# kennychenfs/KataCoffee

Measured on AMD Instinct MI355X. Metric: self-play training rows/sec + MCTS playouts/sec, 5x5 Coffee b6c96 @600 visits, higher is better.
Workload: dtype fp16

## Files before the change

### katacoffee_amd/csrc/search.hip

```cpp
#include <hip/hip_runtime.h>
#include <hip/hip_ext.h>

#include <type_traits>

#include "detmath.h"
#include "engine.h"
#include "kc_board.h"
#include "search.h"

namespace kc {

static constexpr int SVB_IDX_MOVE1 = MAX_P + 1;
static constexpr int SVB_IDX_PLA = 2 * (MAX_P + 1);
static constexpr int SVB_IDX_PAT = 2 * (MAX_P + 1) + 3;
static constexpr int BIG = 0x7fffffff;

KC_D int64_t svbQ(float x) { return llrintf(x * 4294967296.0f); }
KC_D float svbF(int64_t v) { return (float)v * (1.0f / 4294967296.0f); }

KC_D void waveSync() {
  __builtin_amdgcn_wave_barrier();
  asm volatile("" ::: "memory");
}

#ifdef KC_SEARCH_PROFILE
constexpr int SPROF_N = 48;
constexpr int SPROF_MAXG = 16384;
__device__ unsigned long long g_searchProf[SPROF_MAXG * SPROF_N];
__device__ unsigned long long* g_probeKeys = nullptr;
__device__ unsigned long long g_probeMask = 0;
KC_D void probeLeafKey(uint64_t k0, uint64_t k1) {
  if(!g_probeKeys)
    return;
  uint64_t key = (k0 ^ (k1 * 0x9e3779b97f4a7c15ULL)) | 1ull;
  uint64_t i = (key >> 7) & g_probeMask;
  for(int probe = 0; probe < 64; probe++, i = (i + 1) & g_probeMask) {
    const unsigned long long prev = atomicCAS(&g_probeKeys[i], 0ull, (unsigned long long)key);
    if(prev == 0ull)
      return;
    if(prev == key) {
      atomicAdd(&g_searchProf[9], 1ull);
      return;
    }
  }
}
KC_D unsigned long long* sprofLds() {
  __shared__ unsigned long long c[SPROF_N];
  return c;
}
#define SPROF_NOW() clock64()
#define SPROF_WAIT() __builtin_amdgcn_s_waitcnt(0)
#define SPROF_INIT()                   \
  do {                                 \
    if(laneId() < SPROF_N)             \
      sprofLds()[laneId()] = 0;        \
    __syncthreads();                   \
  } while(0)
#define SPROF_ADD(i, v)                                 \
  do {                                                  \
    if(laneId() == 0)                                   \
      sprofLds()[(i)] += (unsigned long long)(v);       \
  } while(0)
#define SPROF_FLUSH()                                                           \
  do {                                                                          \
    __syncthreads();                                                            \
    if(blockIdx.x < SPROF_MAXG && (laneId() < 24 || (laneId() >= 32 && laneId() < 40))) \
      g_searchProf[blockIdx.x * SPROF_N + laneId()] += sprofLds()[laneId()];    \
  } while(0)
#define SPROF_MAX(i, v)                                                                   \
  do {                                                                                    \
    if(laneId() == 0 && blockIdx.x < SPROF_MAXG) {                                        \
      unsigned long long* q_ = &g_searchProf[blockIdx.x * SPROF_N + (i)];                 \
      const unsigned long long v_ = (unsigned long long)(v);                              \
      if(v_ > *q_)                                                                        \
        *q_ = v_;                                                                         \
    }                                                                                     \
  } while(0)
#else
#define SPROF_NOW() 0ull
#define SPROF_WAIT() \
  do {               \
  } while(0)
#define SPROF_INIT() \
  do {               \
  } while(0)
#define SPROF_ADD(i, v) \
  do {                  \
  } while(0)
#define SPROF_MAX(i, v) \
  do {                  \
  } while(0)
#define SPROF_FLUSH() \
  do {                \
  } while(0)
#endif

struct NodeEdges {
  Edge* inl;
  Edge* pool;
  KC_D Edge& operator[](int i) const { return i < INLINE_EDGES ? inl[i] : pool[i - INLINE_EDGES]; }
};

struct GV {
  const SearchDev& d;
  const DTables& T;
  int g, lane;
  const SP* sp;
  const Unc* unc;
  mutable int esel = 0;
  int row;
  int32_t* wpn = nullptr;
  int32_t* wps = nullptr;
  KC_D GV(const SearchDev& d_, int g_) : d(d_), T(*d_.T), g(g_), lane(laneId()), sp(&d_.sp), unc(&d_.unc), row(g_) {}
  KC_D GV(const SearchDev& d_, const DTables& t_, int g_)
      : d(d_), T(t_), g(g_), lane(laneId()), sp(&d_.sp), unc(&d_.unc), row(g_) {}
  KC_D void setDescent(int j) {
    row = g * d.wideK + j;
    wpn = d.widePathNode + (size_t)row * MAX_DEPTH;
    wps = d.widePathSlot + (size_t)row * MAX_DEPTH;
  }
  KC_D Node* nodes() const { return d.nodes + (size_t)g * d.cap; }
  KC_D Edge* inlineEdges(int n) const { return d.edges + ((size_t)g * d.cap + n) * INLINE_EDGES; }
  KC_D Edge* edgePool() const { return d.edgePool + ((size_t)g * 2 + esel) * d.edgePoolCap; }
  KC_D void setEdgeSel(int sel) const { esel = __builtin_amdgcn_readfirstlane(sel); }
  KC_D NodeEdges edges(int n, uint32_t ebase) const { return NodeEdges{inlineEdges(n), edgePool() + ebase}; }
  KC_D NodeEdges edges(int n) const { return edges(n, nodes()[n].edgeBase); }
  KC_D uint64_t* nodeKey(int n) const { return d.nodeKey + ((size_t)g * d.cap + n) * 2; }
  KC_D float* pol(int n) const { return d.policy + ((size_t)g * d.cap + n) * d.P; }
  KC_D uint32_t* freeList() const { return d.freeList + (size_t)g * d.cap; }
  KC_D uint32_t* allocBits() const { return d.allocBits + (size_t)g * (d.cap / 32); }
  KC_D uint64_t* ttKey() const { return d.ttKey + (size_t)g * d.ttCap * 2; }
  KC_D int32_t* ttNode() const { return d.ttNode + (size_t)g * d.ttCap; }
  KC_D size_t svbBase(int sel) const { return ((size_t)g * 2 + sel) * d.svbCap; }
  KC_D float* accPolicy() const { return d.accPolicy + (size_t)g * d.P; }
  KC_D float* rawPolicy() const { return d.rawPolicy + (size_t)g * d.P; }
  KC_D float* rootNoised() const { return d.rootNoised + (size_t)g * d.P; }
  KC_D int32_t* pathNode() const { return wpn ? wpn : d.pathNode + (size_t)g * MAX_DEPTH; }
  KC_D int32_t* pathSlot() const { return wps ? wps : d.pathSlot + (size_t)g * MAX_DEPTH; }
  KC_D TurnRec* turns() const { return d.turns + (size_t)g * d.maxTurns; }
  KC_D int16_t* turnPol(int t) const { return d.turnPol + ((size_t)g * d.maxTurns + t) * d.P; }
};

static_assert(sizeof(GameDev) % 4 == 0, "GameDev copy granularity");
KC_D void storeGame(const GV& v, const GameDev& s) {
  waveSync();
  const uint32_t* src = reinterpret_cast<const uint32_t*>(&s);
  uint32_t* dst = reinterpret_cast<uint32_t*>(&v.d.games[v.g]);
  for(int i = v.lane; i < (int)(sizeof(GameDev) / 4); i += 64)
    dst[i] = src[i];
}

KC_D int sideOf(const SearchDev& d, int g, const GameDev& s) {
  return matchNet(d.slotBase + g, s.gameNum, s.root.pla);
}

template <bool MATCH = false>
KC_D void bindGame(GV& v, const GameDev& s) {
  v.sp = __builtin_amdgcn_readfirstlane(s.noNoise) ? &v.d.spCheap : &v.d.sp;
  if constexpr(MATCH) {
    if(v.d.matchPerSide && __builtin_amdgcn_readfirstlane(sideOf(v.d, v.g, s))) {
      v.sp = &v.d.sp1;
      v.unc = &v.d.unc1;
    }
  }
  v.setEdgeSel(s.edgeSel);
}

KC_D const Expl& explOf(const GV& v) { return v.unc == &v.d.unc1 ? v.d.ex1 : v.d.ex; }
KC_D const RootSearch& rootSearchOf(const GV& v) { return v.unc == &v.d.unc1 ? v.d.rs1 : v.d.rs; }

template <bool MATCH>
KC_D void matchMoveLimits(const GV& v, GameDev& s) {
  if constexpr(MATCH) {
    if(v.d.matchPerSide && __builtin_amdgcn_readfirstlane(sideOf(v.d, v.g, s)))
      s.visitLimit = v.d.sp1.maxVisits;
  }
}

template <bool MATCH = false>
KC_D void loadGame(GV& v, GameDev& s) {
  const uint32_t* src = reinterpret_cast<const uint32_t*>(&v.d.games[v.g]);
  uint32_t* dst = reinterpret_cast<uint32_t*>(&s);
  for(int i = v.lane; i < (int)(sizeof(GameDev) / 4); i += 64)
    dst[i] = src[i];
  waveSync();
  bindGame<MATCH>(v, s);
}

template <int NI>
KC_D float tsum(const float (&x)[NI], int n, int lane) {
  float a = 0.0f;
#pragma unroll
  for(int j = 0; j < NI; j++) {
    int i = lane + 64 * j;
    if(i < n)
      a = j == 0 ? x[j] : a + x[j];
  }
  return waveSum(a);
}

KC_D int bcastI(int v, int srcLane) { return bcastLane(v, srcLane); }

constexpr int SPEC_EDGES = INLINE_EDGES;
template <int NI>
constexpr bool W1_OF = NI <= 4;
KC_D int firstLane(uint64_t m) { return __builtin_ctzll(m); }

KC_D float childWeight(uint32_t edgeVisits, uint32_t childVisits, float rawWeight) {
  return rawWeight * ((float)edgeVisits / (float)(childVisits > 1u ? childVisits : 1u));
}

constexpr int PROBE_W = 16;
KC_D int ttFind(const GV& v, uint64_t k0, uint64_t k1, int& emptySlot) {
  const int mask = v.d.ttCap - 1;
  const int start = (int)(k0 & (uint64_t)mask);
  const uint64_t* key = v.ttKey();
  const int32_t* node = v.ttNode();
  emptySlot = -1;
  const bool act = v.lane < PROBE_W;
  for(int base = 0; base < v.d.ttCap; base += PROBE_W) {
    int s = (start + base + v.lane) & mask;
    const int nd = act ? node[s] : 0;
    const uint64_t ka = act ? key[2 * s] : 0ull, kb = act ? key[2 * s + 1] : 0ull;
    bool match = act && nd >= 0 && ka == k0 && kb == k1;
    uint64_t m = ballot(act && (nd < 0 || match));
    if(m) {
      int f = firstLane(m);
      emptySlot = bcastI(s, f);
      return bcastI(match ? nd : -1, f);
    }
  }
  return -1;
}

KC_D void ttInsertAt(const GV& v, int slot, uint64_t k0, uint64_t k1, int nodeIdx) {
  if(slot >= 0 && v.lane == 0) {
    v.ttKey()[2 * slot] = k0;
    v.ttKey()[2 * slot + 1] = k1;
    v.ttNode()[slot] = nodeIdx;
  }
}

KC_D uint64_t svbProbe(const GV& v, int sel, uint64_t k) {
  const int mask = v.d.svbCap - 1;
  return v.lane < PROBE_W ? v.d.svbKey[v.svbBase(sel) + (((int)(k & (uint64_t)mask) + v.lane) & mask)] : 0ull;
}
KC_D int svbFindOrInsert(const GV& v, int sel, uint64_t k, uint64_t first) {
  const int mask = v.d.svbCap - 1;
  const size_t b = v.svbBase(sel);
  const int start = (int)(k & (uint64_t)mask);
  const bool act = v.lane < PROBE_W;
  for(int base = 0; base < v.d.svbCap; base += PROBE_W) {
    int s = (start + base + v.lane) & mask;
    uint64_t kk = base == 0 ? first : (act ? v.d.svbKey[b + s] : 0ull);
    uint64_t m = ballot(act && (kk == 0 || kk == k));
    if(m) {
      int f = firstLane(m);
      int slot = bcastI(s, f);
      bool empty = bcastLane((int)(kk == 0), f) != 0;
      if(empty && v.lane == f) {
        v.d.svbKey[b + slot] = k;
        v.d.svbD[b + slot] = 0;
        v.d.svbW[b + slot] = 0;
      }
      return slot;
    }
  }
  return -1;
}

template <bool W1 = false>
KC_D uint64_t svbKeyOf(const GV& v, const DBoard& before, int parentPrevPos, int movePos, int mover) {
  const DTables& T = v.T;
  uint64_t h = 0;
  if(v.lane < 25) {
    int wy = v.lane / 5, wx = v.lane % 5;
    int cell = movePos % T.A;
    int xx = cell % T.X + wx - 2, yy = cell / T.X + wy - 2;
    int col = (xx >= 0 && xx < T.X && yy >= 0 && yy < T.Y) ? colorAt<W1>(before, yy * T.X + xx) : 3;
    h = T.svbZ[SVB_IDX_PAT + col * 25 + wy * 5 + wx];
  }
  h = waveXor64(h);
  h ^= T.svbZ[parentPrevPos] ^ T.svbZ[SVB_IDX_MOVE1 + movePos] ^ T.svbZ[SVB_IDX_PLA + mover];
  return h != 0 ? h : 1;
}

KC_D int allocNode(const GV& v, GameDev& s, int nextPla, uint64_t k0, uint64_t k1, bool terminal, int freeIdx = -1) {
  if(s.freeTop <= 0) {
    s.err = ERR_NODE_POOL;
    return -1;
  }
  s.freeTop--;
  int idx = freeIdx >= 0 ? freeIdx : (int)v.freeList()[s.freeTop];
  if(v.lane == 0) {
    Node n;
    n.visits = 0;
    n.weightSum = n.weightSqSum = n.utilityAvg = n.utilitySqAvg = n.winLossAvg = 0.0f;
    n.nnWin = n.nnLoss = n.lastSvbDelta = n.lastSvbWeight = 0.0f;
    n.svbEntry = -1;
    n.numChildren = 0;
    n.nextPla = (uint8_t)nextPla;
    n.flags = terminal ? 2 : 0;
    n.nextPrior = -1.0f;
    n.nextPos = 0xFFFF;
    n.virtualLosses = 0;
    n.edgeBase = 0;
    n.nnWeight = 1.0f;
    v.nodes()[idx] = n;
    v.nodeKey(idx)[0] = k0;
    v.nodeKey(idx)[1] = k1;
    atomicOr(&v.allocBits()[idx >> 5], 1u << (idx & 31));
  }
  s.liveCount++;
  return idx;
}

struct NStats {
  uint32_t visits;
  float weightSum, weightSqSum, utilityAvg, utilitySqAvg, winLossAvg;
};

KC_D NStats addLeafValue(const GV& v, const GameDev& s, int ni, float wl, float weight, bool isTerminal,
                         bool assumeNoExisting) {
  const SP& sp = *v.sp;
  Node* np = &v.nodes()[ni];
  const int svbEntry = np->svbEntry;
  uint32_t visits = np->visits;
  float weightSum = np->weightSum, weightSqSum = np->weightSqSum;
  float utilityAvg = np->utilityAvg, utilitySqAvg = np->utilitySqAvg, winLossAvg = np->winLossAvg;
  float utility = wl;
  if(sp.svbFactor != 0.0f && !isTerminal && svbEntry >= 0) {
    size_t e = v.svbBase(s.svbSel) + svbEntry;
    float dd = svbF(v.d.svbD[e]), ww = svbF(v.d.svbW[e]);
    if(ww > 0.001f)
      utility = utility + (sp.svbFactor * dd) / ww;
  }
  float usq = utility * utility;
  if(assumeNoExisting) {
    winLossAvg = wl;
    utilityAvg = utility;
    utilitySqAvg = usq;
    weightSqSum = weight * weight;
    weightSum = weight;
    visits += 1;
  } else {
    float oldW = weightSum, newW = oldW + weight;
    winLossAvg = (winLossAvg * oldW + wl * weight) / newW;
    utilityAvg = (utilityAvg * oldW + utility * weight) / newW;
    utilitySqAvg = (utilitySqAvg * oldW + usq * weight) / newW;
    weightSqSum = weightSqSum + weight * weight;
    weightSum = newW;
    visits += 1;
  }
  waveSync();
  if(v.lane == 0) {
    np->visits = visits;
    np->weightSum = weightSum;
    np->weightSqSum = weightSqSum;
    np->utilityAvg = utilityAvg;
    np->utilitySqAvg = utilitySqAvg;
    np->winLossAvg = winLossAvg;
  }
  waveSync();
  return NStats{visits, weightSum, weightSqSum, utilityAvg, utilitySqAvg, winLossAvg};
}

KC_D float cdfT(const DTables& T, float z) {
  float dd = (1999.0f * (z - (-50.0f))) / 100.0f;
  if(dd <= 0.0f)
    return 0.0f;
  int idx = (int)dd;
  if(idx >= 1999)
    return 1.0f;
  float lambda = dd - (float)idx;
  float y0 = T.cdf[idx], y1 = T.cdf[idx + 1];
  return y0 + lambda * (y1 - y0);
}

template <int NI, bool EXPL>
struct PathPriors {};
template <int NI>
struct PathPriors<NI, true> {
  float epr[NI];
};
template <int NI, bool EXPL = false>
struct PathLevel : PathPriors<NI, EXPL> {
  int ni, slot, k, nextPla, svbEntry;
  uint32_t ebase;
  float nnWin, nnLoss, nnWeight, lastSvbDelta, lastSvbWeight;
  uint32_t visits0;
  uint32_t ech[NI], evis[NI];
  uint32_t cv[NI];
  float cws[NI], cwsq[NI], cu[NI], cusq[NI], cwl[NI];
  int64_t svbD0, svbW0;
};
struct LevelOut {
  NStats st;
  int svbEntry;
  int64_t svbD, svbW;
};

template <int NI, bool EXPL>
KC_D void loadLevel(const GV& v, int ni, int slot, PathLevel<NI, EXPL>& L) {
  const Node nd = v.nodes()[ni];
  const Edge* E = v.inlineEdges(ni);
  const Edge e0 = v.lane < SPEC_EDGES && v.lane < v.d.P ? E[v.lane] : Edge{0u, 0u, 0.0f, 0u};
  L.ebase = nd.edgeBase;
  L.ech[0] = e0.child;
  L.evis[0] = e0.visits;
  L.ni = ni;
  L.slot = slot;
  L.k = nd.numChildren;
  L.nextPla = nd.nextPla;
  L.svbEntry = nd.svbEntry;
  L.nnWin = nd.nnWin;
  L.nnLoss = nd.nnLoss;
  L.nnWeight = nd.nnWeight;
  L.lastSvbDelta = nd.lastSvbDelta;
  L.lastSvbWeight = nd.lastSvbWeight;
  L.visits0 = nd.visits;
}

template <int NI, bool EXPL>
KC_D void loadKids(const GV& v, const GameDev& s, PathLevel<NI, EXPL>& L) {
  const SP& sp = *v.sp;
  const NodeEdges E = v.edges(L.ni, L.ebase);
  const Node* NS = v.nodes();
#pragma unroll
  for(int j = 0; j < NI; j++) {
    const int i = v.lane + 64 * j;
    L.cv[j] = 0;
    L.cws[j] = L.cwsq[j] = L.cu[j] = L.cusq[j] = L.cwl[j] = 0.0f;
    if constexpr(EXPL)
      L.epr[j] = 0.0f;
    if(j > 0 || i >= SPEC_EDGES)
      L.ech[j] = L.evis[j] = 0u;
    if(i < L.k) {
      if(j > 0 || i >= SPEC_EDGES) {
        const Edge e = E[i];
        L.ech[j] = e.child;
        L.evis[j] = e.visits;
      }
      if constexpr(EXPL) {
        const Edge e = E[i];
        L.epr[j] = L.ni == s.rootIdx ? v.rootNoised()[e.move] : e.prior;
      }
      const Node& c = NS[L.ech[j]];
      L.cv[j] = c.visits;
      L.cws[j] = c.weightSum;
      L.cwsq[j] = c.weightSqSum;
      L.cu[j] = c.utilityAvg;
      L.cusq[j] = c.utilitySqAvg;
      L.cwl[j] = c.winLossAvg;
    }
  }
  const size_t e = v.svbBase(s.svbSel) + (L.svbEntry >= 0 ? L.svbEntry : 0);
  L.svbD0 = v.d.svbD[e];
  L.svbW0 = v.d.svbW[e];
  (void)sp;
}

template <int NI, bool EXPL, class F>
KC_D LevelOut computeLevel(const GV& v, const GameDev& s, PathLevel<NI, EXPL>& L, const LevelOut& below, bool haveBelow,
                           int numVisitsToAdd, bool isRoot, F&& issueNext) {
  const SP& sp = *v.sp;
  const unsigned long long tLoads = SPROF_NOW();
  (void)tLoads;
  SPROF_WAIT();
  const unsigned long long tCalc = SPROF_NOW();
  (void)tCalc;
  SPROF_ADD(36, tCalc - tLoads);
  SPROF_ADD(39, 1);
  const int k = L.k, slot = L.slot;
  const int nextPla = L.nextPla;
  const int svbEntry = L.svbEntry;
  const NodeEdges E = v.edges(L.ni, L.ebase);
  const bool svbOn = sp.svbFactor != 0.0f && svbEntry >= 0;
  int64_t svbD0 = L.svbD0, svbW0 = L.svbW0;
  if(svbOn && haveBelow && below.svbEntry == svbEntry) {
    svbD0 = below.svbD;
    svbW0 = below.svbW;
  }
  bool good[NI];
  float wAdj[NI], selfU[NI], cU[NI], cUsq[NI], cWl[NI], cWs[NI], cWsq[NI], tmp[NI];
  int numGood = 0;
  float maxW = 0.0f;
#pragma unroll
  for(int j = 0; j < NI; j++) {
    int i = v.lane + 64 * j;
    good[j] = false;
    wAdj[j] = selfU[j] = cU[j] = cUsq[j] = cWl[j] = cWs[j] = cWsq[j] = 0.0f;
    if(i < k) {
      uint32_t evis = L.evis[j];
      uint32_t cv = L.cv[j];
      float ws = L.cws[j], wsq = L.cwsq[j], u = L.cu[j], usq = L.cusq[j], wl = L.cwl[j];
      if(i == slot) {
        evis += 1;
        E[i].visits = evis;
        if(haveBelow) {
          cv = below.st.visits;
          ws = below.st.weightSum;
          wsq = below.st.weightSqSum;
          u = below.st.utilityAvg;
          usq = below.st.utilitySqAvg;
          wl = below.st.winLossAvg;
        }
      }
      good[j] = cv > 0 && ws > 0.0f && evis > 0;
      if(good[j]) {
        cU[j] = u;
        cUsq[j] = usq;
        cWl[j] = wl;
        cWs[j] = ws;
        cWsq[j] = wsq;
        selfU[j] = nextPla == 2 ? cU[j] : -cU[j];
        wAdj[j] = childWeight(evis, cv, ws);
        maxW = wAdj[j] > maxW ? wAdj[j] : maxW;
      }
    }
    numGood += __popcll(ballot(good[j]));
  }
  maxW = waveMax(maxW);
  const float origTotal = tsum<NI>(wAdj, k, v.lane);
  float currentTotal = origTotal;
  bool pruning = false;
  if constexpr(EXPL) {
    const Expl& ex = explOf(v);
    pruning = ex.noisePruning != 0;
    if(pruning && pruneNoiseApplies(numGood, origTotal)) {
      PruneScan sc{0.0f, 0.0f, 0.0f};
#pragma unroll
      for(int j = 0; j < NI; j++) {
        const int cnt = k - 64 * j < 64 ? k - 64 * j : 64;
        const uint64_t gm = ballot(good[j]);
        for(int l = 0; l < cnt; l++) {
          if(!((gm >> l) & 1ull))
            continue;
          const float old = bcastLaneF(wAdj[j], l), u = bcastLaneF(selfU[j], l), pr = bcastLaneF(L.epr[j], l);
          const float nw = pruneNoiseStep(ex, sc, old, u, pr);
          if(v.lane == l)
            wAdj[j] = nw;
        }
      }
      currentTotal = sc.wSum;
    }
  }
  float amountToSubtract = 0.0f, amountToPrune = 0.0f;
  if(isRoot && sp.rootNoise && !pruning) {
    amountToSubtract = fminf(sp.moveSubtract, maxW / 64.0f);
    amountToPrune = fminf(sp.movePrune, maxW / 64.0f);
  }
  if(numGood > 0 && currentTotal > 0.0f) {
    float stdev[NI];
#pragma unroll
    for(int j = 0; j < NI; j++) {
      if(j > 0 && 64 * j >= k) {
        stdev[j] = tmp[j] = 0.0f;
        continue;
      }
      stdev[j] = good[j] ? sqrtf(1e-8f + 1.0f / (1.5f * sqrtf(wAdj[j]))) : 0.0f;
      tmp[j] = good[j] ? selfU[j] * wAdj[j] : 0.0f;
    }
    const float simpleValue = tsum<NI>(tmp, k, v.lane) / currentTotal;
    float y0[NI], y1[NI], lam[NI], pc[NI];
    int mode[NI];
#pragma unroll
    for(int j = 0; j < NI; j++) {
      mode[j] = 0;
      y0[j] = y1[j] = lam[j] = pc[j] = 0.0f;
      if(j > 0 && 64 * j >= k)
        continue;
      if(!good[j] || wAdj[j] < amountToPrune)
        continue;
      float z = (selfU[j] - simpleValue) / stdev[j];
      float dd = (1999.0f * (z - (-50.0f))) / 100.0f;
      if(dd <= 0.0f) {
        mode[j] = 2;
        pc[j] = 0.0f;
        continue;
      }
      int idx = (int)dd;
      if(idx >= 1999) {
        mode[j] = 2;
        pc[j] = 1.0f;
        continue;
      }
      mode[j] = 1;
      lam[j] = dd - (float)idx;
      y0[j] = v.T.cdf[idx];
      y1[j] = v.T.cdf[idx + 1];
    }
    issueNext();
#pragma unroll
    for(int j = 0; j < NI; j++) {
      if((j > 0 && 64 * j >= k) || mode[j] == 0) {
        tmp[j] = 0.0f;
        continue;
      }
      float nw = wAdj[j] - amountToSubtract;
      if(nw <= 0.0f)
        nw = 0.0f;
      const float c = mode[j] == 1 ? y0[j] + lam[j] * (y1[j] - y0[j]) : pc[j];
      float p = c + 0.0001f;
      float f = sp.valueWeightExp == 0.5f ? sqrtf(p) : dpow(p, sp.valueWeightExp);
      tmp[j] = nw * f;
    }
    const float totalNew = tsum<NI>(tmp, k, v.lane);
    const float factor = currentTotal / totalNew;
#pragma unroll
    for(int j = 0; j < NI; j++)
      wAdj[j] = tmp[j] * factor;
  } else {
    issueNext();
  }
  float wlv[NI], uv[NI], usqv[NI], wsqv[NI];
#pragma unroll
  for(int j = 0; j < NI; j++) {
    if((j > 0 && 64 * j >= k) || !good[j]) {
      wlv[j] = uv[j] = usqv[j] = wsqv[j] = 0.0f;
      continue;
    }
    float ws = wAdj[j] / cWs[j];
    wlv[j] = wAdj[j] * cWl[j];
    uv[j] = wAdj[j] * cU[j];
    usqv[j] = wAdj[j] * cUsq[j];
    wsqv[j] = (ws * ws) * cWsq[j];
  }
  float winLossSum = tsum<NI>(wlv, k, v.lane);
  float utilitySum = tsum<NI>(uv, k, v.lane);
  float utilitySqSum = tsum<NI>(usqv, k, v.lane);
  float weightSqSum = tsum<NI>(wsqv, k, v.lane);
  float weightSum = currentTotal;
  float wl = L.nnWin - L.nnLoss;
  float utility = wl;
  float newLastD = L.lastSvbDelta, newLastW = L.lastSvbWeight;
  LevelOut out;
  out.svbEntry = -1;
  out.svbD = out.svbW = 0;
  if(svbOn) {
    int64_t D = svbD0, Wt = svbW0;
    if(currentTotal > 1e-10f) {
      float utilityChildren = utilitySum / currentTotal;
      float svbWv = dpow(origTotal, sp.svbExp);
      float svbDv = (utilityChildren - utility) * svbWv;
      D += svbQ(svbDv) - svbQ(L.lastSvbDelta);
      Wt += svbQ(svbWv) - svbQ(L.lastSvbWeight);
      waveSync();
      if(v.lane == 0) {
        const size_t e = v.svbBase(s.svbSel) + svbEntry;
        v.d.svbD[e] = D;
        v.d.svbW[e] = Wt;
      }
      newLastD = svbDv;
      newLastW = svbWv;
      out.svbEntry = svbEntry;
      out.svbD = D;
      out.svbW = Wt;
    }
    float dd = svbF(D), ww = svbF(Wt);
    if(ww > 0.001f)
      utility = utility + (sp.svbFactor * dd) / ww;
  }
  const float selfW = L.nnWeight;
  winLossSum = winLossSum + wl * selfW;
  utilitySum = utilitySum + utility * selfW;
  utilitySqSum = utilitySqSum + (utility * utility) * selfW;
  weightSqSum = weightSqSum + selfW * selfW;
  weightSum = weightSum + selfW;
  out.st.winLossAvg = winLossSum / weightSum;
  out.st.utilityAvg = utilitySum / weightSum;
  out.st.utilitySqAvg = utilitySqSum / weightSum;
  out.st.weightSqSum = weightSqSum;
  out.st.weightSum = weightSum;
  out.st.visits = L.visits0 + (uint32_t)numVisitsToAdd;
  waveSync();
  const unsigned long long tStore = SPROF_NOW();
  (void)tStore;
  SPROF_ADD(37, tStore - tCalc);
  if(v.lane == 0) {
    Node* np = &v.nodes()[L.ni];
    np->winLossAvg = out.st.winLossAvg;
    np->utilityAvg = out.st.utilityAvg;
    np->utilitySqAvg = out.st.utilitySqAvg;
    np->weightSqSum = out.st.weightSqSum;
    np->weightSum = out.st.weightSum;
    np->visits = out.st.visits;
    np->lastSvbDelta = newLastD;
    np->lastSvbWeight = newLastW;
  }
  waveSync();
  SPROF_ADD(38, SPROF_NOW() - tStore);
  return out;
}

template <int NI, bool EXPL = false>
KC_D void backupPath(const GV& v, const GameDev& s, int pathLen, NStats leaf, bool haveLeaf) {
  const int32_t* pn = v.pathNode();
  const int32_t* ps = v.pathSlot();
  const int myNode = v.lane < pathLen ? pn[v.lane] : 0, mySlot = v.lane < pathLen ? ps[v.lane] : 0;
  auto nodeAt = [&](int j) { return j < 64 ? bcastLane(myNode, j) : pn[j]; };
  auto slotAt = [&](int j) { return j < 64 ? bcastLane(mySlot, j) : ps[j]; };
  if(pathLen <= 0)
    return;
  LevelOut below;
  bool haveBelow = haveLeaf;
  below.st = leaf;
  below.svbEntry = -1;
  below.svbD = below.svbW = 0;
  int j = pathLen - 1;
  if constexpr(NI > 2) {
    for(; j >= 0; j--) {
      PathLevel<NI, EXPL> cur;
      loadLevel<NI, EXPL>(v, nodeAt(j), slotAt(j), cur);
      loadKids<NI, EXPL>(v, s, cur);
      below = computeLevel<NI, EXPL>(v, s, cur, below, haveBelow, 1, cur.ni == s.rootIdx, [] {});
      haveBelow = true;
    }
    return;
  }
  PathLevel<NI, EXPL> cur, nxt;
  loadLevel<NI, EXPL>(v, nodeAt(j), slotAt(j), cur);
  if(j > 0)
    loadLevel<NI, EXPL>(v, nodeAt(j - 1), slotAt(j - 1), nxt);
  loadKids<NI, EXPL>(v, s, cur);
  for(; j >= 0; j--) {
    PathLevel<NI, EXPL> nn;
    auto issueNext = [&] {
      if(j > 0)
        loadKids<NI, EXPL>(v, s, nxt);
      if(j > 1)
        loadLevel<NI, EXPL>(v, nodeAt(j - 2), slotAt(j - 2), nn);
    };
    below = computeLevel<NI, EXPL>(v, s, cur, below, haveBelow, 1, cur.ni == s.rootIdx, issueNext);
    haveBelow = true;
    if(j > 0) {
      cur = nxt;
      nxt = nn;
    }
  }
}

KC_D float fpuValue(const SP& sp, const Node& n, int pla, bool isRoot, float probMass) {
  float parentUtility = n.utilityAvg;
  float forFpu = parentUtility;
  if(sp.fpuByVisited) {
    float pw = sp.fpuByVisitedPow == 2.0f ? probMass * probMass : dpow(probMass, sp.fpuByVisitedPow);
    float avgWeight = fminf(1.0f, pw);
    forFpu = avgWeight * parentUtility + (1.0f - avgWeight) * (n.nnWin - n.nnLoss);
  }
  float redMax = isRoot ? sp.rootFpuRedMax : sp.fpuRedMax;
  float lossProp = isRoot ? sp.rootFpuLossProp : sp.fpuLossProp;
  float reduction = redMax * sqrtf(probMass);
  float fpu = pla == 2 ? forFpu - reduction : forFpu + reduction;
  float lossValue = pla == 2 ? -1.0f : 1.0f;
  fpu = fpu + (lossValue - fpu) * lossProp;
  return fpu;
}

KC_D float exploreScaling(const SP& sp, float totalChildWeight) {
  float c = sp.cpuct;
  if(sp.cpuctLog != 0.0f)
    c = c + sp.cpuctLog * dlog((totalChildWeight + sp.cpuctBase) / sp.cpuctBase);
  return c * sqrtf(totalChildWeight + 0.01f);
}

template <int NI, bool EXPL = false, bool VL = false>
KC_D int selectBest(const GV& v, const GameDev& s, int ni, const Node& n, const float* pol, bool isRoot, int& newPos,
                    uint32_t* hasBits, const Edge& e0, Edge& ce, uint32_t& cVisits, uint32_t& cFlags) {
  const SP& sp = *v.sp;
  const int P = v.d.P;
  const int k = n.numChildren;
  const int pla = n.nextPla;
  if(isRoot) {
    for(int w = v.lane; w < (P + 31) / 32; w += 64)
      hasBits[w] = 0;
    waveSync();
  }
  const unsigned long long tKids = SPROF_NOW();
  (void)tKids;
  const NodeEdges E = v.edges(ni, n.edgeBase);
  const Node* NS = v.nodes();
  float probs[NI], cw[NI], pv[NI], cu[NI];
  uint32_t cvis[NI], cfl[NI];
  [[maybe_unused]] uint32_t cvl[NI];
  Edge ev[NI];
#pragma unroll
  for(int j = 0; j < NI; j++) {
    int i = v.lane + 64 * j;
    probs[j] = cw[j] = pv[j] = cu[j] = 0.0f;
    cvis[j] = cfl[j] = 0;
    if constexpr(VL)
      cvl[j] = 0;
    ev[j] = Edge{0u, 0u, 0.0f, 0u};
    if(j > 0 && 64 * j >= k)
      continue;
    if(i < k) {
      const Edge e = j == 0 && i < SPEC_EDGES ? e0 : E[i];
      ev[j] = e;
      const Node& c = NS[e.child];
      float p = isRoot ? pol[e.move] : e.prior;
      cvis[j] = c.visits;
      cfl[j] = c.flags;
      if constexpr(VL)
        cvl[j] = c.virtualLosses;
      cu[j] = c.utilityAvg;
      pv[j] = p;
      probs[j] = p < 0.0f ? 0.0f : p;
      cw[j] = p < 0.0f ? 0.0f : childWeight(e.visits, cvis[j], c.weightSum);
      if(isRoot)
        atomicOr(&hasBits[e.move >> 5], 1u << (e.move & 31));
    }
  }
  SPROF_WAIT();
  const unsigned long long tArith = SPROF_NOW();
  (void)tArith;
  SPROF_ADD(33, tArith - tKids);
  const float probMass = tsum<NI>(probs, k, v.lane);
  const float total = tsum<NI>(cw, k, v.lane);
  const float fpu = fpuValue(sp, n, pla, isRoot, probMass);
  float scaling = exploreScaling(sp, total);
  if constexpr(EXPL)
    scaling = scaling * exploreStdevFactor(explOf(v), n.visits, n.weightSum, n.utilityAvg, n.utilitySqAvg);
  float rsWide = 0.0f, rsThr = 0.0f, rsMaxW = 0.0f, rsWpv = 0.0f, rsLeft = 0.0f;
  uint64_t rsKey = 0;
  if constexpr(EXPL) {
    if(isRoot) {
      const RootSearch& rs = rootSearchOf(v);
      rsWide = rs.wide;
      rsThr = rs.thr;
      if(rsWide > 0.0f)
        rsKey = wideRootKey(s.rngSeed, s.root.turn, n.visits);
      if(rsThr > 0.0f) {
        float m = 0.0f;
#pragma unroll
        for(int j = 0; j < NI; j++)
          m = fmaxf(m, cw[j]);
        rsMaxW = waveMax(m);
        rsWpv = n.weightSum / (float)n.visits;
        rsLeft = (float)(s.visitLimit - (int32_t)n.visits);
      }
    }
  }
  float best = -__builtin_inff();
  int bestIdx = BIG;
#pragma unroll
  for(int j = 0; j < NI; j++) {
    int i = v.lane + 64 * j;
    if((j > 0 && 64 * j >= k) || i >= k)
      continue;
    float p = pv[j];
    float val;
    if(p < 0.0f)
      val = -__builtin_inff();
    else {
      float w = cw[j];
      float u = (cvis[j] == 0 || w <= 0.0f) ? fpu : cu[j];
      if constexpr(VL)
        virtualLossAdjust(v.d.vlPerThread, cvl[j], pla, u, w);
      bool futile = false;
      if constexpr(EXPL)
        futile = rsThr > 0.0f && futileChild(rsThr, rsMaxW, rsWpv, rsLeft, ev[j].visits, cvis[j], w);
      if(futile)
        val = FUTILE_VALUE;
      else if(isRoot && sp.rootDesiredCoeff > 0.0f && p > 0.0f && w < sqrtf((p * total) * sp.rootDesiredCoeff))
        val = 1e20f;
      else {
        if constexpr(EXPL) {
          if(rsWide > 0.0f) {
            u = wideUtility(u, wideBonus(rsWide, rsKey, (int)ev[j].move), pla);
            p = wideSmoothedPrior(rsWide, p);
          }
        }
        val = (scaling * p) / (1.0f + w) + (pla == 2 ? u : -u);
      }
    }
    if(val > best) {
      best = val;
      bestIdx = i;
    }
  }
  waveArgmax(best, bestIdx);
  int bestSlot = best > -__builtin_inff() ? bestIdx : -1;
  if(bestSlot >= 0) {
    Edge me{0u, 0u, 0.0f, 0u};
    uint32_t mv = 0, mf = 0;
#pragma unroll
    for(int j = 0; j < NI; j++)
      if(j == (bestSlot >> 6)) {
        me = ev[j];
        mv = cvis[j];
        mf = cfl[j];
      }
    const int bl = bestSlot & 63;
    ce.child = (uint32_t)bcastLane((int)me.child, bl);
    ce.visits = (uint32_t)bcastLane((int)me.visits, bl);
    ce.move = (uint32_t)bcastLane((int)me.move, bl);
    ce.prior = 0.0f;
    cVisits = (uint32_t)bcastLane((int)mv, bl);
    cFlags = (uint32_t)bcastLane((int)mf, bl);
  }
  float bp = -1.0f;
  int bpos = BIG;
  if(isRoot) {
    waveSync();
    for(int pos = v.lane; pos < P; pos += 64) {
      if((hasBits[pos >> 5] >> (pos & 31)) & 1u)
        continue;
      float p = pol[pos];
      if(p < 0.0f)
        continue;
      if(p > bp) {
        bp = p;
        bpos = pos;
      }
    }
    waveArgmax(bp, bpos);
  } else if(n.nextPos != 0xFFFF) {
    bp = n.nextPrior;
    bpos = n.nextPos;
  }
  newPos = -1;
  if(bpos != BIG) {
    float val;
    bool futile = false;
    if constexpr(EXPL)
      futile = rsThr > 0.0f && futileNew(rsThr, rsMaxW, rsWpv, rsLeft);
    if(futile)
      val = FUTILE_VALUE;
    else {
      float u = fpu;
      if constexpr(EXPL) {
        if(rsWide > 0.0f) {
          u = wideUtility(u, wideBonus(rsWide, rsKey, bpos), pla);
          bp = wideSmoothedPrior(rsWide, bp);
        }
      }
      val = (scaling * bp) / 1.0f + (pla == 2 ? u : -u);
    }
    if(val > best) {
      bestSlot = k;
      newPos = bpos;
    }
  }
  SPROF_ADD(34, SPROF_NOW() - tArith);
  return bestSlot;
}

template <int NI>
KC_D void nextExpansion(const GV& v, const float (&pv)[NI], float curPrior, int curPos, float& nPrior, int& nPos) {
  const int P = v.d.P;
  float best = -1.0f;
  int bi = BIG;
#pragma unroll
  for(int j = 0; j < NI; j++) {
    const int p = v.lane + 64 * j;
    const float x = pv[j];
    if(p < P && x >= 0.0f && (x < curPrior || (x == curPrior && p > curPos)) && x > best) {
      best = x;
      bi = p;
    }
  }
  waveArgmax(best, bi);
  nPrior = bi != BIG ? best : -1.0f;
  nPos = bi != BIG ? bi : 0xFFFF;
}

KC_D void addVirtualLoss(const GV& v, int node) {
  waveSync();
  if(v.lane == 0)
    v.nodes()[node].virtualLosses += 1;
}
KC_D void removeVirtualLosses(const GV& v, int pathLen, int last) {
  waveSync();
  const int32_t* pn = v.pathNode();
  for(int i = v.lane; i < pathLen; i += 64)
    v.nodes()[i + 1 < pathLen ? pn[i + 1] : last].virtualLosses -= 1;
  waveSync();
}

template <bool VL>
KC_D void pushLevel(GameDev& s) {
  if constexpr(VL) {
    const int len = s.pathLen + 1;
    waveSync();
    s.pathLen = len;
    waveSync();
  } else {
    s.pathLen++;
  }
}

template <int NI, bool EXPL = false, bool VL = false>
KC_D void descend(const GV& v, GameDev& s, uint32_t* hasBits, float* rootPol , bool loadRootPol = true) {
  constexpr bool W1 = W1_OF<NI>;
  const SP& sp = *v.sp;
  const DTables& T = v.T;
  s.pathLen = 0;
  DBoard b = s.root;
  int ni = s.rootIdx;
  uint32_t scanned = 0;
  auto loadE0 = [&](int node) {
    return v.lane < SPEC_EDGES && v.lane < v.d.P ? v.inlineEdges(node)[v.lane] : Edge{0u, 0u, 0.0f, 0u};
  };
  Edge e0 = loadE0(ni);
  Node n = v.nodes()[ni];
  const int freeIdx = s.freeTop > 0 ? (int)v.freeList()[s.freeTop - 1] : -1;
  if(!VL || loadRootPol) {
    const float* rn = v.rootNoised();
    float pr[NI];
#pragma unroll
    for(int j = 0; j < NI; j++) {
      const int p = v.lane + 64 * j;
      pr[j] = p < v.d.P ? rn[p] : 0.0f;
    }
#pragma unroll
    for(int j = 0; j < NI; j++) {
      const int p = v.lane + 64 * j;
      if(p < v.d.P)
        rootPol[p] = pr[j];
    }
    waveSync();
  }
  while(true) {
    {
      const unsigned long long tw = SPROF_NOW();
      (void)tw;
      SPROF_WAIT();
      SPROF_ADD(32, SPROF_NOW() - tw);
      SPROF_ADD(35, 1);
    }
    if(n.flags & 2) {
      s.leafKind = LEAF_TERMINAL;
      s.leafNode = ni;
      s.leaf = b;
      break;
    }
    const bool isRoot = ni == s.rootIdx;
    const float* pol = isRoot ? rootPol : v.pol(ni);
    int newPos = -1;
    scanned += n.numChildren;
    const unsigned long long tSel = SPROF_NOW();
// ... 3722 lines not shown
```

Measured before the change: 29520.

## Hoist path-backup context and make child loads branchless for prefetch overlap

```diff
diff --git a/katacoffee_amd/csrc/search.hip b/katacoffee_amd/csrc/search.hip
--- a/katacoffee_amd/csrc/search.hip
+++ b/katacoffee_amd/csrc/search.hip
@@ -22,6 +22,7 @@
   __builtin_amdgcn_wave_barrier();
   asm volatile("" ::: "memory");
 }
+constexpr int WAIT_VMCNT0 = 0x0F70;
 
 #ifdef KC_SEARCH_PROFILE
 constexpr int SPROF_N = 48;
@@ -50,6 +51,7 @@
 }
 #define SPROF_NOW() clock64()
 #define SPROF_WAIT() __builtin_amdgcn_s_waitcnt(0)
+#define SPROF_PIN(x) asm volatile("" : "+v"(x))
 #define SPROF_INIT()                   \
   do {                                 \
     if(laneId() < SPROF_N)             \
@@ -64,7 +66,7 @@
 #define SPROF_FLUSH()                                                           \
   do {                                                                          \
     __syncthreads();                                                            \
-    if(blockIdx.x < SPROF_MAXG && (laneId() < 24 || (laneId() >= 32 && laneId() < 40))) \
+    if(blockIdx.x < SPROF_MAXG && (laneId() < 24 || (laneId() >= 32 && laneId() < 42))) \
       g_searchProf[blockIdx.x * SPROF_N + laneId()] += sprofLds()[laneId()];    \
   } while(0)
 #define SPROF_MAX(i, v)                                                                   \
@@ -79,6 +81,9 @@
 #else
 #define SPROF_NOW() 0ull
 #define SPROF_WAIT() \
+  do {               \
+  } while(0)
+#define SPROF_PIN(x) \
   do {               \
   } while(0)
 #define SPROF_INIT() \
@@ -400,11 +405,46 @@
   int64_t svbD, svbW;
 };
 
+struct PathCtx {
+  Node* nodes;
+  Edge* inl;
+  Edge* pool;
+  int64_t *svbD, *svbW;
+  const float* cdf;
+  const float* rootNoised;
+  const Expl* ex;
+  int lane, rootIdx;
+  float svbFactor, svbExp, valueWeightExp, moveSubtract, movePrune;
+  int rootNoise;
+  KC_D NodeEdges edges(int n, uint32_t ebase) const { return NodeEdges{inl + (size_t)n * INLINE_EDGES, pool + ebase}; }
+};
+KC_D PathCtx pathCtx(const GV& v, const GameDev& s) {
+  const SP& sp = *v.sp;
+  const size_t sb = v.svbBase(__builtin_amdgcn_readfirstlane(s.svbSel));
+  PathCtx c;
+  c.nodes = v.nodes();
+  c.inl = v.inlineEdges(0);
+  c.pool = v.edgePool();
+  c.svbD = v.d.svbD + sb;
+  c.svbW = v.d.svbW + sb;
+  c.cdf = v.T.cdf;
+  c.rootNoised = v.rootNoised();
+  c.ex = &explOf(v);
+  c.lane = v.lane;
+  c.rootIdx = __builtin_amdgcn_readfirstlane(s.rootIdx);
+  c.svbFactor = sp.svbFactor;
+  c.svbExp = sp.svbExp;
+  c.valueWeightExp = sp.valueWeightExp;
+  c.moveSubtract = sp.moveSubtract;
+  c.movePrune = sp.movePrune;
+  c.rootNoise = sp.rootNoise;
+  return c;
+}
+
 template <int NI, bool EXPL>
-KC_D void loadLevel(const GV& v, int ni, int slot, PathLevel<NI, EXPL>& L) {
-  const Node nd = v.nodes()[ni];
-  const Edge* E = v.inlineEdges(ni);
-  const Edge e0 = v.lane < SPEC_EDGES && v.lane < v.d.P ? E[v.lane] : Edge{0u, 0u, 0.0f, 0u};
+KC_D void loadLevel(const PathCtx& c, int ni, int slot, PathLevel<NI, EXPL>& L) {
+  const Node nd = c.nodes[ni];
+  const Edge e0 = (c.inl + (size_t)ni * INLINE_EDGES)[c.lane < SPEC_EDGES ? c.lane : 0];
   L.ebase = nd.edgeBase;
   L.ech[0] = e0.child;
   L.evis[0] = e0.visits;
@@ -422,48 +462,56 @@
 }
 
 template <int NI, bool EXPL>
-KC_D void loadKids(const GV& v, const GameDev& s, PathLevel<NI, EXPL>& L) {
-  const SP& sp = *v.sp;
-  const NodeEdges E = v.edges(L.ni, L.ebase);
-  const Node* NS = v.nodes();
+KC_D void loadKids(const PathCtx& c, PathLevel<NI, EXPL>& L) {
+  const NodeEdges E = c.edges(L.ni, L.ebase);
+  const int k = L.k;
 #pragma unroll
   for(int j = 0; j < NI; j++) {
-    const int i = v.lane + 64 * j;
-    L.cv[j] = 0;
-    L.cws[j] = L.cwsq[j] = L.cu[j] = L.cusq[j] = L.cwl[j] = 0.0f;
-    if constexpr(EXPL)
-      L.epr[j] = 0.0f;
-    if(j > 0 || i >= SPEC_EDGES)
-      L.ech[j] = L.evis[j] = 0u;
-    if(i < L.k) {
-      if(j > 0 || i >= SPEC_EDGES) {
-        const Edge e = E[i];
-        L.ech[j] = e.child;
-        L.evis[j] = e.visits;
-      }
-      if constexpr(EXPL) {
-        const Edge e = E[i];
-        L.epr[j] = L.ni == s.rootIdx ? v.rootNoised()[e.move] : e.prior;
-      }
-      const Node& c = NS[L.ech[j]];
-      L.cv[j] = c.visits;
-      L.cws[j] = c.weightSum;
-      L.cwsq[j] = c.weightSqSum;
-      L.cu[j] = c.utilityAvg;
-      L.cusq[j] = c.utilitySqAvg;
-      L.cwl[j] = c.winLossAvg;
-    }
-  }
-  const size_t e = v.svbBase(s.svbSel) + (L.svbEntry >= 0 ? L.svbEntry : 0);
-  L.svbD0 = v.d.svbD[e];
-  L.svbW0 = v.d.svbW[e];
-  (void)sp;
+    const int i = c.lane + 64 * j;
+    uint32_t ch = j == 0 ? L.ech[0] : 0u, ev = j == 0 ? L.evis[0] : 0u;
+    const bool late = i >= SPEC_EDGES && i < k;
+    if(ballot(late)) {
+      const Edge e = E[late ? i : 0];
+      ch = late ? e.child : ch;
+      ev = late ? e.visits : ev;
+    }
+    L.ech[j] = ch;
+    L.evis[j] = ev;
+    const Node& cn = c.nodes[i < k ? ch : (uint32_t)L.ni];
+    L.cv[j] = cn.visits;
+    L.cws[j] = cn.weightSum;
+    L.cwsq[j] = cn.weightSqSum;
+    L.cu[j] = cn.utilityAvg;
+    L.cusq[j] = cn.utilitySqAvg;
+    L.cwl[j] = cn.winLossAvg;
+  }
+  const int se = L.svbEntry >= 0 ? L.svbEntry : 0;
+  L.svbD0 = c.svbD[se];
+  L.svbW0 = c.svbW[se];
+  if constexpr(EXPL) {
+    float pr[NI];
+    uint32_t mv[NI];
+#pragma unroll
+    for(int j = 0; j < NI; j++) {
+      const int i = c.lane + 64 * j;
+      const Edge e = E[i < k ? i : 0];
+      pr[j] = e.prior;
+      mv[j] = e.move;
+    }
+    if(L.ni == c.rootIdx) {
+#pragma unroll
+      for(int j = 0; j < NI; j++)
+        pr[j] = c.rootNoised[mv[j]];
+    }
+#pragma unroll
+    for(int j = 0; j < NI; j++)
+      L.epr[j] = pr[j];
+  }
 }
 
 template <int NI, bool EXPL, class F>
-KC_D LevelOut computeLevel(const GV& v, const GameDev& s, PathLevel<NI, EXPL>& L, const LevelOut& below, bool haveBelow,
+KC_D LevelOut computeLevel(const PathCtx& c, const PathLevel<NI, EXPL>& L, const LevelOut& below, bool haveBelow,
                            int numVisitsToAdd, bool isRoot, F&& issueNext) {
-  const SP& sp = *v.sp;
   const unsigned long long tLoads = SPROF_NOW();
   (void)tLoads;
   SPROF_WAIT();
@@ -474,8 +522,8 @@
   const int k = L.k, slot = L.slot;
   const int nextPla = L.nextPla;
   const int svbEntry = L.svbEntry;
-  const NodeEdges E = v.edges(L.ni, L.ebase);
-  const bool svbOn = sp.svbFactor != 0.0f && svbEntry >= 0;
+  const NodeEdges E = c.edges(L.ni, L.ebase);
+  const bool svbOn = c.svbFactor != 0.0f && svbEntry >= 0;
   int64_t svbD0 = L.svbD0, svbW0 = L.svbW0;
   if(svbOn && haveBelow && below.svbEntry == svbEntry) {
     svbD0 = below.svbD;
@@ -487,7 +535,7 @@
   float maxW = 0.0f;
 #pragma unroll
   for(int j = 0; j < NI; j++) {
-    int i = v.lane + 64 * j;
+    int i = c.lane + 64 * j;
     good[j] = false;
     wAdj[j] = selfU[j] = cU[j] = cUsq[j] = cWl[j] = cWs[j] = cWsq[j] = 0.0f;
     if(i < k) {
@@ -521,11 +569,11 @@
     numGood += __popcll(ballot(good[j]));
   }
   maxW = waveMax(maxW);
-  const float origTotal = tsum<NI>(wAdj, k, v.lane);
+  const float origTotal = tsum<NI>(wAdj, k, c.lane);
   float currentTotal = origTotal;
   bool pruning = false;
   if constexpr(EXPL) {
-    const Expl& ex = explOf(v);
+    const Expl& ex = *c.ex;
     pruning = ex.noisePruning != 0;
     if(pruning && pruneNoiseApplies(numGood, origTotal)) {
       PruneScan sc{0.0f, 0.0f, 0.0f};
@@ -538,7 +586,7 @@
             continue;
           const float old = bcastLaneF(wAdj[j], l), u = bcastLaneF(selfU[j], l), pr = bcastLaneF(L.epr[j], l);
           const float nw = pruneNoiseStep(ex, sc, old, u, pr);
-          if(v.lane == l)
+          if(c.lane == l)
             wAdj[j] = nw;
         }
       }
@@ -546,9 +594,9 @@
     }
   }
   float amountToSubtract = 0.0f, amountToPrune = 0.0f;
-  if(isRoot && sp.rootNoise && !pruning) {
-    amountToSubtract = fminf(sp.moveSubtract, maxW / 64.0f);
-    amountToPrune = fminf(sp.movePrune, maxW / 64.0f);
+  if(isRoot && c.rootNoise && !pruning) {
+    amountToSubtract = fminf(c.moveSubtract, maxW / 64.0f);
+    amountToPrune = fminf(c.movePrune, maxW / 64.0f);
   }
   if(numGood > 0 && currentTotal > 0.0f) {
     float stdev[NI];
@@ -561,7 +609,7 @@
       stdev[j] = good[j] ? sqrtf(1e-8f + 1.0f / (1.5f * sqrtf(wAdj[j]))) : 0.0f;
       tmp[j] = good[j] ? selfU[j] * wAdj[j] : 0.0f;
     }
-    const float simpleValue = tsum<NI>(tmp, k, v.lane) / currentTotal;
+    const float simpleValue = tsum<NI>(tmp, k, c.lane) / currentTotal;
     float y0[NI], y1[NI], lam[NI], pc[NI];
     int mode[NI];
 #pragma unroll
@@ -587,10 +635,15 @@
       }
       mode[j] = 1;
       lam[j] = dd - (float)idx;
-      y0[j] = v.T.cdf[idx];
-      y1[j] = v.T.cdf[idx + 1];
-    }
+      y0[j] = c.cdf[idx];
+      y1[j] = c.cdf[idx + 1];
+    }
+    const unsigned long long tIssue = SPROF_NOW();
+    (void)tIssue;
     issueNext();
+    const unsigned long long tIssued = SPROF_NOW();
+    (void)tIssued;
+    SPROF_ADD(40, tIssued - tIssue);
 #pragma unroll
     for(int j = 0; j < NI; j++) {
       if((j > 0 && 64 * j >= k) || mode[j] == 0) {
@@ -600,12 +653,14 @@
       float nw = wAdj[j] - amountToSubtract;
       if(nw <= 0.0f)
         nw = 0.0f;
-      const float c = mode[j] == 1 ? y0[j] + lam[j] * (y1[j] - y0[j]) : pc[j];
-      float p = c + 0.0001f;
-      float f = sp.valueWeightExp == 0.5f ? sqrtf(p) : dpow(p, sp.valueWeightExp);
+      const float cd = mode[j] == 1 ? y0[j] + lam[j] * (y1[j] - y0[j]) : pc[j];
+      float p = cd + 0.0001f;
+      float f = c.valueWeightExp == 0.5f ? sqrtf(p) : dpow(p, c.valueWeightExp);
       tmp[j] = nw * f;
     }
-    const float totalNew = tsum<NI>(tmp, k, v.lane);
+    SPROF_PIN(tmp[0]);
+    SPROF_ADD(41, SPROF_NOW() - tIssued);
+    const float totalNew = tsum<NI>(tmp, k, c.lane);
     const float factor = currentTotal / totalNew;
 #pragma unroll
     for(int j = 0; j < NI; j++)
@@ -626,10 +681,10 @@
     usqv[j] = wAdj[j] * cUsq[j];
     wsqv[j] = (ws * ws) * cWsq[j];
   }
-  float winLossSum = tsum<NI>(wlv, k, v.lane);
-  float utilitySum = tsum<NI>(uv, k, v.lane);
-  float utilitySqSum = tsum<NI>(usqv, k, v.lane);
-  float weightSqSum = tsum<NI>(wsqv, k, v.lane);
+  float winLossSum = tsum<NI>(wlv, k, c.lane);
+  float utilitySum = tsum<NI>(uv, k, c.lane);
+  float utilitySqSum = tsum<NI>(usqv, k, c.lane);
+  float weightSqSum = tsum<NI>(wsqv, k, c.lane);
   float weightSum = currentTotal;
   float wl = L.nnWin - L.nnLoss;
   float utility = wl;
@@ -641,15 +696,14 @@
     int64_t D = svbD0, Wt = svbW0;
     if(currentTotal > 1e-10f) {
       float utilityChildren = utilitySum / currentTotal;
-      float svbWv = dpow(origTotal, sp.svbExp);
+      float svbWv = dpow(origTotal, c.svbExp);
       float svbDv = (utilityChildren - utility) * svbWv;
       D += svbQ(svbDv) - svbQ(L.lastSvbDelta);
       Wt += svbQ(svbWv) - svbQ(L.lastSvbWeight);
       waveSync();
-      if(v.lane == 0) {
-        const size_t e = v.svbBase(s.svbSel) + svbEntry;
-        v.d.svbD[e] = D;
-        v.d.svbW[e] = Wt;
+      if(c.lane == 0) {
+        c.svbD[svbEntry] = D;
+        c.svbW[svbEntry] = Wt;
       }
       newLastD = svbDv;
       newLastW = svbWv;
@@ -659,7 +713,7 @@
     }
     float dd = svbF(D), ww = svbF(Wt);
     if(ww > 0.001f)
-      utility = utility + (sp.svbFactor * dd) / ww;
+      utility = utility + (c.svbFactor * dd) / ww;
   }
   const float selfW = L.nnWeight;
   winLossSum = winLossSum + wl * selfW;
@@ -677,8 +731,8 @@
   const unsigned long long tStore = SPROF_NOW();
   (void)tStore;
   SPROF_ADD(37, tStore - tCalc);
-  if(v.lane == 0) {
-    Node* np = &v.nodes()[L.ni];
+  if(c.lane == 0) {
+    Node* np = &c.nodes[L.ni];
     np->winLossAvg = out.st.winLossAvg;
     np->utilityAvg = out.st.utilityAvg;
     np->utilitySqAvg = out.st.utilitySqAvg;
@@ -702,6 +756,7 @@
   auto slotAt = [&](int j) { return j < 64 ? bcastLane(mySlot, j) : ps[j]; };
   if(pathLen <= 0)
     return;
+  const PathCtx c = pathCtx(v, s);
   LevelOut below;
   bool haveBelow = haveLeaf;
   below.st = leaf;
@@ -711,32 +766,36 @@
   if constexpr(NI > 2) {
     for(; j >= 0; j--) {
       PathLevel<NI, EXPL> cur;
-      loadLevel<NI, EXPL>(v, nodeAt(j), slotAt(j), cur);
-      loadKids<NI, EXPL>(v, s, cur);
-      below = computeLevel<NI, EXPL>(v, s, cur, below, haveBelow, 1, cur.ni == s.rootIdx, [] {});
+      loadLevel<NI, EXPL>(c, nodeAt(j), slotAt(j), cur);
+      loadKids<NI, EXPL>(c, cur);
+      below = computeLevel<NI, EXPL>(c, cur, below, haveBelow, 1, cur.ni == c.rootIdx, [] {});
       haveBelow = true;
     }
     return;
   }
-  PathLevel<NI, EXPL> cur, nxt;
-  loadLevel<NI, EXPL>(v, nodeAt(j), slotAt(j), cur);
+  PathLevel<NI, EXPL> cur, nxt, nn;
+  loadLevel<NI, EXPL>(c, nodeAt(j), slotAt(j), cur);
   if(j > 0)
-    loadLevel<NI, EXPL>(v, nodeAt(j - 1), slotAt(j - 1), nxt);
-  loadKids<NI, EXPL>(v, s, cur);
-  for(; j >= 0; j--) {
-    PathLevel<NI, EXPL> nn;
+    loadLevel<NI, EXPL>(c, nodeAt(j - 1), slotAt(j - 1), nxt);
+  loadKids<NI, EXPL>(c, cur);
+  __builtin_amdgcn_s_waitcnt(WAIT_VMCNT0);
+  auto level = [&](PathLevel<NI, EXPL>& lc, PathLevel<NI, EXPL>& ln, PathLevel<NI, EXPL>& la)
+                   __attribute__((always_inline)) {
     auto issueNext = [&] {
       if(j > 0)
-        loadKids<NI, EXPL>(v, s, nxt);
+        loadKids<NI, EXPL>(c, ln);
       if(j > 1)
-        loadLevel<NI, EXPL>(v, nodeAt(j - 2), slotAt(j - 2), nn);
+        loadLevel<NI, EXPL>(c, nodeAt(j - 2), slotAt(j - 2), la);
     };
-    below = computeLevel<NI, EXPL>(v, s, cur, below, haveBelow, 1, cur.ni == s.rootIdx, issueNext);
+    below = computeLevel<NI, EXPL>(c, lc, below, haveBelow, 1, lc.ni == c.rootIdx, issueNext);
     haveBelow = true;
-    if(j > 0) {
-      cur = nxt;
-      nxt = nn;
-    }
+    return --j < 0;
+  };
+  for(;;) {
+    if(level(cur, nxt, nn))
+      break;
+    cur = nxt;
+    nxt = nn;
   }
 }
 
```

New measurement: 29880, median of 6. 1.01x the previous value.
